# sota-zk-labs/zkp-implementation

Measured on AMD Instinct MI355X. Metric: G1 MSM scalar-muls/sec, higher is better.
Workload: dtype u32 (unsaturated 28-bit-limb Montgomery, 381-bit Fq; 64-bit accumulate)

## Files before the change

zkp-implementation_amd/csrc/api.hip:

```cpp
#include <hip/hip_runtime.h>

#include <algorithm>
#include <array>
#include <atomic>
#include <chrono>
#include <cstdio>
#include <cstdlib>
#include <cstring>
#include <condition_variable>
#include <functional>
#include <map>
#include <memory>
#include <mutex>
#include <new>
#include <string>
#include <thread>
#include <tuple>
#include <vector>

#include "../../include/zkp_hip.h"
#include "host_ff.hpp"
#include "kzg_host.hpp"
#include "msm.hpp"
#include "ntt.hpp"
// ... 225 lines not shown
    Stream stream;
    Stream copy_stream;
    Stream sort_stream;
    Stream xstream;
    Event ws_event;
    hipStream_t ws_stream = nullptr;
    bool ws_pending = false;
    std::vector<ProfRec> prof;
    hipStream_t prof_last = nullptr;
    std::map<std::pair<int, int>, DevBuf> radix_tw[2];
    std::map<std::pair<unsigned, int>, NttPlan<Fr>> plans_fr;
    std::map<std::pair<unsigned, int>, NttPlan<Gl>> plans_gl;
    static constexpr int COSET_WAYS = 8;
    CosetCache<Fr> coset_fr[COSET_WAYS];
    CosetCache<Gl> coset_gl[COSET_WAYS];
    unsigned coset_victim[2] = {0, 0};
    DevBuf ntt_scratch;
    std::map<std::pair<unsigned, int>, DevBuf> axis0_tw[2];
    DevBuf scalars, over;
    TypedBuf<uint32_t> digits, sorted, counts, start, perm, result;
    TypedBuf<uint2> entries;
    TypedBuf<uint4> pieces, buckets, parts, pyr1, odd0, odd1;
    PinnedBuf host_result;
    PinnedBuf fri_small;
    DevBuf fb_table;
    bool fb_ready = false;
    DevBuf tmp;
    Event copy_event;
    std::vector<Event> copy_events;
    Event ev_sort[2], ev_acc[2], ev_begin;
    DevBuf fri_arena, fri_meta;
    DevBuf clk;
    uint32_t tail_max_waves = 2048;
    DevBuf xchg_a, xchg_b;
    std::vector<Event> xev;
    bool peers_enabled = false;
    ~Ctx() {
        std::lock_guard<std::mutex> lk(mu);
        (void)hipSetDevice(device);
        (void)hipDeviceSynchronize();
    }
};
enum { CLK_MSM_ACCUMULATE = 0, CLK_MAD_PROBE = 1, CLK_NTT_FR = 2, CLK_NTT_GL = 3, CLK_COUNT = 4 };
static const char* const kClkNames[CLK_COUNT] = {"msm_accumulate", "mad_probe", "ntt_fr_pass", "ntt_gl_pass"};

struct Runtime {
    std::mutex mu;
    std::vector<std::unique_ptr<Ctx>> slots;
    bool multi = false;
};
Runtime& g_rt = *new Runtime;

ClkRec* clk_record(int which) {
    if (!g_prof_on.load(std::memory_order_relaxed)) return nullptr;
    Ctx& c = ctx();
    if (!c.clk.p) {
        if (c.clk.ensure(sizeof(ClkRec) * CLK_COUNT) != ZKP_OK) return nullptr;
        if (hipMemset(c.clk.p, 0, sizeof(ClkRec) * CLK_COUNT) != hipSuccess) return nullptr;
    }
    return reinterpret_cast<ClkRec*>(c.clk.p) + which;
}
thread_local int t_slot = -1;
thread_local Ctx* t_cur = nullptr;
Ctx& ctx() { return *t_cur; }
std::vector<ProfRec>& prof_records() { return ctx().prof; }
hipStream_t& prof_last_stream() { return ctx().prof_last; }
// ... 640 lines not shown
            cnt++;
        }
    }
    *total_ms = tot;
    *count = cnt;
    return ZKP_OK;
} ZKP_CATCH_INT
const char* zkp_last_error(void) { return g_err.c_str(); }

}

namespace {

int create_slot_locked(int device) {
    int count = 0;
    if (hipGetDeviceCount(&count) != hipSuccess || count == 0) return fail(ZKP_E_DEVICE, "no HIP device visible");
    if (device < 0 || device >= count) return fail(ZKP_E_ARG, "device index out of range");
    hipDeviceProp_t prop;
    HIPCHK(hipGetDeviceProperties(&prop, device));
    if (std::strncmp(prop.gcnArchName, "gfx950", 6) != 0)
        return fail(ZKP_E_DEVICE, std::string("device is ") + prop.gcnArchName + ", this library is built for gfx950 only");
    HIPCHK(hipSetDevice(device));
    ZCHK(allow_big_lds((ntt_pass_strided<Fr, NttOps<Fr>::LOG_T>)));
    ZCHK(allow_big_lds((ntt_pass_strided<Fr, NttOps<Fr>::LOG_T - 1>)));
    ZCHK(allow_big_lds((ntt_pass_strided<Fr, NttOps<Fr>::LOG_T - 2>)));
    ZCHK(allow_big_lds((ntt_pass_strided<Gl, NttOps<Gl>::LOG_T>)));
    ZCHK(allow_big_lds(ntt_pass_last<Fr>));
    ZCHK(allow_big_lds(ntt_pass_last<Gl>));
    ZCHK(allow_big_lds(msm_partscatter_kernel<PS_TILE_BIG>));
    ZCHK(allow_big_lds(msm_partscatter_kernel<PS_TILE_MID>));
    ZCHK(allow_big_lds(msm_partscatter_kernel<PS_TILE_SMALL>));
    ZCHK(allow_big_lds(fri_tail_kernel<FriGl>));
    ZCHK(allow_big_lds(fri_tail_kernel<FriFr>));
    auto c = std::make_unique<Ctx>();
    c->device = device;
    c->slot = (int)g_rt.slots.size();
    {
        int per_cu = 0;
        uint32_t cap = (uint32_t)prop.multiProcessorCount * 4 * 2;
        if (hipOccupancyMaxActiveBlocksPerMultiprocessor(&per_cu, msm_pyramid_tail_kernel, (int)PYR_TAIL_THREADS, 0) == hipSuccess && per_cu > 0)
            cap = std::min<uint32_t>(cap, (uint32_t)per_cu * (uint32_t)prop.multiProcessorCount * (PYR_TAIL_THREADS / 64));
        else
            (void)hipGetLastError();
        c->tail_max_waves = std::max<uint32_t>(cap, 4);
    }
    if (c->stream.make(hipStreamNonBlocking) != hipSuccess) return fail(ZKP_E_DEVICE, "hipStreamCreate failed");
    g_rt.slots.push_back(std::move(c));
    return ZKP_OK;
}

}

extern "C" {

int zkp_init(int device) try {
    std::lock_guard<std::mutex> g(g_rt.mu);
    if (!g_rt.slots.empty()) return ZKP_OK;
    if (device < 0 && hipGetDevice(&device) != hipSuccess) device = 0;
    return create_slot_locked(device);
} ZKP_CATCH_INT

int zkp_init_devices(const int* devices, int n_devices) try {
    if (n_devices < 0 || n_devices > 64) return fail(ZKP_E_ARG, "n_devices out of range");
    std::lock_guard<std::mutex> g(g_rt.mu);
    std::vector<int> want;
    if (n_devices == 0 || !devices) {
        int count = 0;
        if (hipGetDeviceCount(&count) != hipSuccess || count == 0) return fail(ZKP_E_DEVICE, "no HIP device visible");
// ... 756 lines not shown
```

zkp-implementation_amd/csrc/g1_28.hpp:

```cpp
#pragma once
#include "fq28.hpp"

namespace zkp {

struct A28 {
    Fq28 x, y;
    static ZKP_DEV A28 load(const uint4* p) {
        A28 a;
        a.x = Fq28::load(p);
        a.y = Fq28::load(p + 4);
        return a;
    }
    ZKP_DEV void store(uint4* p) const {
        x.store(p);
        y.store(p + 4);
    }
};

struct X28 {
    Fq28 x, y, zz, zzz;
    static ZKP_DEV X28 infinity() {
        X28 r;
        r.x = Fq28::zero(); r.y = Fq28::zero(); r.zz = Fq28::zero(); r.zzz = Fq28::zero();
        return r;
// ... 232 lines not shown
}
template <bool CHAIN = false>
ZKP_DEV void g1_28_add_stream(const uint4* __restrict__ pa, const uint4* __restrict__ pb, uint4* __restrict__ dst, uint64_t st) {
    g1_28_add_stream_body<CHAIN>(pa, pb, dst, st);
}
template <bool CHAIN = false>
ZKP_DEV void g1_28_add_stream_inplace(uint4* pa, const uint4* __restrict__ pb, uint64_t st) {
    g1_28_add_stream_body<CHAIN>(pa, pb, pa, st);
}

template <int CTRL>
ZKP_DEV Fq28 quad_perm(const Fq28& v) {
    Fq28 r;
#pragma unroll
    for (int i = 0; i < NL28; i++) r.l[i] = (uint32_t)__builtin_amdgcn_mov_dpp((int)v.l[i], CTRL, 0xf, 0xf, true);
    return r;
}
ZKP_DEV Fq28 quad_bcast(const Fq28& v, int src) {
    switch (src & 3) {
        case 0: return quad_perm<0x00>(v);
        case 1: return quad_perm<0x55>(v);
        case 2: return quad_perm<0xaa>(v);
        default: return quad_perm<0xff>(v);
    }
}
ZKP_DEV Fq28 quad_xor1(const Fq28& v) { return quad_perm<0xb1>(v); }
ZKP_DEV int quad_bcast0(int v) { return __builtin_amdgcn_mov_dpp(v, 0x00, 0xf, 0xf, true); }
ZKP_DEV Fq28 fq28_select(bool c, const Fq28& a, const Fq28& b) {
    Fq28 r;
#pragma unroll
    for (int i = 0; i < NL28; i++) r.l[i] = c ? a.l[i] : b.l[i];
    return r;
}
ZKP_DEV void g1_28_add_quad(const uint4* srcA, const uint4* __restrict__ srcB, uint4* dst, uint64_t stride, int j) {
    const bool odd = (j & 1) != 0, hi = (j & 2) != 0;
    const uint4* mine = odd ? srcB : srcA;
    const uint4* other = odd ? srcA : srcB;
    const int zf = hi ? 12 : 8;
    const Fq28 xy = Fq28::load_s(mine + (hi ? 4 : 0) * stride, stride);
    const Fq28 zo = Fq28::load_s(other + zf * stride, stride);
    const Fq28 zm = Fq28::load_s(mine + zf * stride, stride);
    const int inf_mine = zm.all_zero() ? 1 : 0, inf_other = zo.all_zero() ? 1 : 0;
    const int inf_a = quad_bcast0(inf_mine), inf_b = quad_bcast0(inf_other);
    const Fq28 m1 = xy * zo;
    const Fq28 d = sub4(quad_xor1(m1), m1);
    const Fq28 m2 = fq28_select(odd, zo, d) * fq28_select(odd, zm, d);
    const Fq28 pp = quad_bcast(m2, 0);
    const int p_zero = quad_bcast0(tight_is_zero_mod_p(m2) ? 1 : 0);
    if (inf_a | inf_b | p_zero) {
        if (j == 0) {
            X28 a = X28::load_s(srcA, stride);
            const X28 b = X28::load_s(srcB, stride);
            g1_28_add(a, b);
            a.store_s(dst, stride);
        }
        return;
    }
    const Fq28 u1 = quad_bcast(m1, 0);
    const Fq28 m3 = fq28_select(hi, u1, fq28_select(odd, m2, d)) * pp;
    const Fq28 ppp = quad_bcast(m3, 0);
    const Fq28 s1 = quad_bcast(m1, 2);
    const Fq28 x3 = normalise(sub8w(sub4(m2, ppp), m3 + m3));
    const Fq28 t = sub16(m3, x3);
    const Fq28 lhs4 = fq28_select(hi, fq28_select(odd, m2, d), s1);
    const Fq28 rhs4 = fq28_select(hi && !odd, t, ppp);
    const Fq28 m4 = lhs4 * rhs4;
    const Fq28 v = quad_bcast(m4, 0);
    if (j == 2) {
        x3.store_s(dst, stride);
        normalise(sub4(m4, v)).store_s(dst + 4 * stride, stride);
    } else if (j == 1) {
        m3.store_s(dst + 8 * stride, stride);
    } else if (j == 3) {
        m4.store_s(dst + 12 * stride, stride);
    }
}

}
```

zkp-implementation_amd/csrc/knobs.hpp:

```cpp
#pragma once
#include <climits>
#include <cstdlib>

namespace zkp {

enum Knob {
    KNOB_MSM_C, KNOB_MSM_FEED_RANGES, KNOB_MSM_FEED_FIRST_PCT, KNOB_MSM_FEED_SECOND_PCT, KNOB_MSM_RANGE_LOG, KNOB_MSM_FIRST_PCT,
    KNOB_MSM_NCHUNK, KNOB_SORT_LO_BITS, KNOB_MSM_NO_OVERLAP, KNOB_MSM_SPLIT_LOG,
    KNOB_MSM_PLAN_END,
    KNOB_FOLD_LANE_MIN = KNOB_MSM_PLAN_END, KNOB_PYR_TAIL_THREADS, KNOB_PYR_TAIL_BLOCKS, KNOB_PYR_TAIL_HALF, KNOB_TEST_TAIL_STARVE,
    KNOB_MSM_NO_POLL, KNOB_POOL_NO_WARM, KNOB_MSM_BALANCE_FROM, KNOB_SRS_EXPAND_MAX_BYTES, KNOB_NTT_TW_MATRIX_MAX_LOG,
    KNOB_NTT_NO_WIDE_PASS, KNOB_NTT_SHARD_MIN_LOG, KNOB_PLONK_NO_POLL, KNOB_FRI_ZERO_AS_0, KNOB_FRI_FR_TAIL_LOG,
    KNOB_COUNT
};

enum KnobKind { KNOB_TUNING, KNOB_POLICY, KNOB_TEST_HOOK };
enum KnobForm {
    KNOB_INT,
    KNOB_INT_CLAMP,
    KNOB_INT_REFUSE,
    KNOB_SET,
    KNOB_ONE
};
constexpr long long KNOB_COMPUTED = LLONG_MIN;

struct KnobRow {
    Knob id;
    const char* name;
    KnobKind kind;
    KnobForm form;
    long long lo, hi, dflt;
    const char* doc;
};

constexpr KnobRow kKnobs[KNOB_COUNT] = {
    {KNOB_MSM_C, "ZKP_MSM_C", KNOB_TUNING, KNOB_INT, 8, 16, KNOB_COMPUTED,
     "window bits of an MSM over unexpanded bases (16 from 2048 terms, else 8): profiles/r01_window_sweep.txt"},
    {KNOB_MSM_FEED_RANGES, "ZKP_MSM_FEED_RANGES", KNOB_TUNING, KNOB_INT, 1, 64, 0,
     "host-fed scalars in this many equal ranges (0: the unequal split): profiles/r04_i_host_scalars_unequal_ranges.md"},
    {KNOB_MSM_FEED_FIRST_PCT, "ZKP_MSM_FEED_FIRST_PCT", KNOB_TUNING, KNOB_INT, 0, 90, KNOB_COMPUTED,
     "share of the first host-fed range (25, from 2^21 terms 10; 0: equal ranges): profiles/r04_i_host_scalars_unequal_ranges.md"},
    {KNOB_MSM_FEED_SECOND_PCT, "ZKP_MSM_FEED_SECOND_PCT", KNOB_TUNING, KNOB_INT, 0, 80, KNOB_COMPUTED,
     "share of a second short host-fed range (30 from 2^21 terms, else none): profiles/r05_o_range_handover.md"},
    {KNOB_MSM_RANGE_LOG, "ZKP_MSM_RANGE_LOG", KNOB_TUNING, KNOB_INT, 10, 30, 0,
     "scalar ranges of at most 2^v terms in shared-bucket mode (0: 2^24, or 2^23 above 12 planes): "
     "profiles/r02_a_accumulate_prefetch_and_range_sweep.md"},
    {KNOB_MSM_FIRST_PCT, "ZKP_MSM_FIRST_PCT", KNOB_TUNING, KNOB_INT, 1, 90, 0,
     "resident scalars, single MSM: a short first range of this share (0: none): profiles/r05_o_range_handover.md"},
    {KNOB_MSM_NCHUNK, "ZKP_MSM_NCHUNK", KNOB_TUNING, KNOB_INT, 1, 4096, 0, "chunks per bucket set of the counting sort (0: 512 over the bucket sets)"},
    {KNOB_SORT_LO_BITS, "ZKP_SORT_LO_BITS", KNOB_TUNING, KNOB_INT, 6, 10, 0,
     "bins of the sort's second pass, 2^v (0: 8..10 by window width): profiles/r04_m_sort_tiles.md"},
    {KNOB_MSM_NO_OVERLAP, "ZKP_MSM_NO_OVERLAP", KNOB_TUNING, KNOB_SET, 0, 1, 0,
     "sort of range r+1 after, not under, the accumulate of range r: profiles/r02_j_sort_under_accumulate.md"},
    {KNOB_MSM_SPLIT_LOG, "ZKP_MSM_SPLIT_LOG", KNOB_TUNING, KNOB_INT, 0, 2, KNOB_COMPUTED,
     "2^v lanes (quads) share a bucket's run in a single-range MSM (default: by bucket count): profiles/r02_n_split_runs.md"},
    {KNOB_FOLD_LANE_MIN, "ZKP_FOLD_LANE_MIN", KNOB_TUNING, KNOB_INT, 0, LLONG_MAX, 1ll << 15,
     "adds in one fold launch from which one lane per add is used: profiles/r05_m_fold_lane.md"},
    {KNOB_PYR_TAIL_THREADS, "ZKP_PYR_TAIL_THREADS", KNOB_TUNING, KNOB_INT_REFUSE, 64, 512, 256,
     "workgroup size of the bucket reduction's last-levels launch, a multiple of 64: profiles/r04_e_bucket_reduce_counters.md"},
    {KNOB_PYR_TAIL_BLOCKS, "ZKP_PYR_TAIL_BLOCKS", KNOB_TUNING, KNOB_INT_REFUSE, 1, 256, 16,
     "workgroups per bucket set of that launch: profiles/r04_e_bucket_reduce_counters.md"},
    {KNOB_PYR_TAIL_HALF, "ZKP_PYR_TAIL_HALF", KNOB_TUNING, KNOB_INT_REFUSE, 1, UINT_MAX, 64,
     "pairs per array from which that launch takes over: profiles/r04_e_bucket_reduce_counters.md"},
    {KNOB_TEST_TAIL_STARVE, "ZKP_TEST_TAIL_STARVE", KNOB_TEST_HOOK, KNOB_SET, 0, 1, 0,
     "every MSM FAILS: the last-levels barrier waits for a workgroup that does not exist (tests/test_gpu_parity.py)"},
    {KNOB_MSM_NO_POLL, "ZKP_MSM_NO_POLL", KNOB_TUNING, KNOB_SET, 0, 1, 0,
     "stream wait instead of polling the MSM's result flags: profiles/r05_k_result_flag_polling.md"},
    {KNOB_POOL_NO_WARM, "ZKP_POOL_NO_WARM", KNOB_TUNING, KNOB_SET, 0, 1, 0,
     "do not wake the host pool before a batch's tails: profiles/r05_q_host_pool_warm.md"},
    {KNOB_MSM_BALANCE_FROM, "ZKP_MSM_BALANCE_FROM", KNOB_TUNING, KNOB_INT, 0, INT_MAX, 1,
     "expansion: slices of floor/ceil(256 / planes) bits from this many bits of overshoot: profiles/r03_j_balanced_slices.md"},
    {KNOB_SRS_EXPAND_MAX_BYTES, "ZKP_SRS_EXPAND_MAX_BYTES", KNOB_POLICY, KNOB_INT, 0, LLONG_MAX, LLONG_MAX,
     "an SRS expansion larger than this is refused with ZKP_E_NOMEM; the bases stay unexpanded"},
    {KNOB_NTT_TW_MATRIX_MAX_LOG, "ZKP_NTT_TW_MATRIX_MAX_LOG", KNOB_TUNING, KNOB_INT_CLAMP, 0, 30, 24,
     "largest transform whose pass-0 twiddles are kept as a matrix: profiles/r02_m_ntt_twiddle_matrix.md"},
    {KNOB_NTT_NO_WIDE_PASS, "ZKP_NTT_NO_WIDE_PASS", KNOB_TUNING, KNOB_SET, 0, 1, 0,
     "no radix-2^9 / 2^10 passes in transform plans built from now on (a plan is cached per size): profiles/r02_l_ntt_wide_pass.md"},
    {KNOB_NTT_SHARD_MIN_LOG, "ZKP_NTT_SHARD_MIN_LOG", KNOB_POLICY, KNOB_INT_CLAMP, 4, INT_MAX, 24,
     "host transforms from 2^v elements are spread over the device slots"},
    {KNOB_PLONK_NO_POLL, "ZKP_PLONK_NO_POLL", KNOB_TUNING, KNOB_SET, 0, 1, 0,
     "stream wait instead of the polled sequence number behind a proof's read-backs: profiles/r05_q_host_pool_warm.md"},
    {KNOB_FRI_ZERO_AS_0, "ZKP_FRI_ZERO_AS_0", KNOB_POLICY, KNOB_ONE, 0, 1, 0,
     "1: a zero field element enters hashes and the transcript as \"0\" instead of the empty string"},
    {KNOB_FRI_FR_TAIL_LOG, "ZKP_FRI_FR_TAIL_LOG", KNOB_TUNING, KNOB_INT_CLAMP, 0, 10, 9,
     "FRI over Fr: layers of up to 2^v points run in the tail kernel (0: none)"},
};

constexpr bool knob_rows_in_enum_order() {
    for (int i = 0; i < KNOB_COUNT; i++)
        if (kKnobs[i].id != i) return false;
    return true;
}
static_assert(knob_rows_in_enum_order(), "kKnobs: one row per enumerator, in the enum's order");

inline long long knob_int(Knob k, long long dflt) {
    const KnobRow& r = kKnobs[k];
// ... 15 lines not shown
```

zkp-implementation_amd/csrc/msm.hpp:

```cpp
#pragma once
#include "g1.hpp"
#include "g1_28.hpp"
#include "fq28_inv.hpp"
#include "msm_plan.hpp"

namespace zkp {

constexpr int MSM_THREADS = 256;
constexpr int ACC_THREADS = 256;
#define ZKP_AT(f, o) offsetof(MsmGeom, f) == o
static_assert(sizeof(MsmGeom) == 152 && ZKP_AT(c, 0) && ZKP_AT(nwin, 4) && ZKP_AT(nb, 8) && ZKP_AT(nchunk, 12) && ZKP_AT(n, 16) && ZKP_AT(chunk, 24) &&
              ZKP_AT(ns, 32) && ZKP_AT(plane_stride, 40) && ZKP_AT(nslice, 48) && ZKP_AT(shared, 52) && ZKP_AT(run_limit, 56) && ZKP_AT(piece, 60) &&
              ZKP_AT(resume, 64) && ZKP_AT(off, 68) && ZKP_AT(interleave, 140) && ZKP_AT(split_log, 144) && ZKP_AT(more, 148), "MsmGeom layout");
#undef ZKP_AT
static_assert(sizeof(SortGeom) == 8 && offsetof(SortGeom, lo_bits) == 0 && offsetof(SortGeom, nhi) == 4, "SortGeom layout");

ZKP_DEV uint64_t bucket_cap(const MsmGeom& g) { return (uint64_t)g.nwin * g.nb; }

#ifdef ZKP_MSM_CHECK
__device__ uint32_t g_msm_check[32];
ZKP_DEV bool msm_check_fail(int cls, uint32_t v0, uint32_t v1) {
    if (atomicAdd(&g_msm_check[cls * 4], 1u) == 0) { g_msm_check[cls * 4 + 1] = v0; g_msm_check[cls * 4 + 2] = v1; }
    return true;
}
// ... 424 lines not shown
        raw.store(planes + (s * plane_stride + i) * 8);
        run.store(slot(s, 2));
        x.zz.store(slot(s, 0));
        x.zzz.store(slot(s, 1));
        run = run * x.zzz;
    }
    Fq28 inv = fq28_inverse_gcd(run);
#pragma unroll 1
    for (uint32_t s = nplanes - 1; s >= 1; s--) {
        const Fq28 zi3 = inv * Fq28::load(slot(s, 2));
        inv = inv * Fq28::load(slot(s, 1));
        const Fq28 zi = zi3 * Fq28::load(slot(s, 0));
        const Fq28 zi2 = zi * zi;
        uint4* dst = planes + (s * plane_stride + i) * 8;
        const A28 raw = A28::load(dst);
        A28 q;
        q.x = raw.x * zi2;
        q.y = raw.y * zi3;
        q.store(dst);
    }
}

ZKP_DEV uint4* split_dst(const MsmGeom& g, uint4* buckets, uint4* parts, uint32_t part) {
    return part ? parts + (uint64_t)(part - 1) * 16 * bucket_cap(g) : buckets;
}
ZKP_DEV void split_run(const MsmGeom& g, uint32_t part, uint32_t& lo, uint32_t& hi) {
    if (!g.split_log) return;
    const uint32_t len = hi - lo;
    hi = lo + (uint32_t)(((uint64_t)len * (part + 1)) >> g.split_log);
    lo = lo + (uint32_t)(((uint64_t)len * part) >> g.split_log);
}


ZKP_DEV uint64_t pyr_pos(uint32_t i, uint32_t n) { return (uint64_t)(i >> 1) + (uint64_t)(i & 1u) * (n >> 1); }

#ifdef ZKP_ACC_PLAIN_PRODUCTS
constexpr bool ACC_CHAIN = false;
#else
constexpr bool ACC_CHAIN = true;
#endif
ZKP_DEV void msm_accumulate_run(const uint4* __restrict__ bases28, const uint32_t* __restrict__ idx, uint32_t lo,
                                uint32_t hi, const MsmGeom& g, uint4* dst, uint64_t dst_stride, bool resume,
                                const uint4* src = nullptr, uint64_t src_stride = 1) {
#ifdef ZKP_MSM_CHECK
    if ((lo > hi || hi > g.n) && msm_check_fail(3, lo, hi)) return;
#endif
    if (resume && lo == hi) {
        if (src != dst) X28::load_s(src, src_stride).store_s(dst, dst_stride);
        return;
    }
    X28 acc = resume ? X28::load_s(src, src_stride) : X28::infinity();
    auto locate = [&](uint32_t e) {
        uint64_t pt = e & 0x7fffffffu;
#ifdef ZKP_MSM_CHECK
        if (pt >= g.n && msm_check_fail(2, e, (uint32_t)g.n)) pt = 0;
#endif
        if (g.shared) {
            const uint32_t ns32 = (uint32_t)g.ns, s = (uint32_t)pt / ns32;
            pt = (uint64_t)s * g.plane_stride + ((uint32_t)pt - s * ns32);
        }
        return bases28 + pt * 8;
    };
    uint32_t k = lo;
    if (!resume && hi - lo >= 2) {
        const uint32_t e0 = idx[k], e1 = idx[k + 1];
        {
            A28 p0 = A28::load(locate(e0));
// ... 249 lines not shown
    const uint4* pw = pieces + (uint64_t)w * desc_cap * 16;
    X28 acc = X28::infinity();
    for (uint32_t p = p0 + lane; p < p1; p += 64) {
        X28 x = X28::load(pw + (uint64_t)p * 16);
        g1_28_add(acc, x);
    }
    for (uint32_t off = 32; off > 0; off >>= 1) {
        acc.store(sh + lane * 16);
        __syncthreads();
        if (lane < off) {
            X28 x = X28::load(sh + (lane + off) * 16);
            g1_28_add(acc, x);
        }
        __syncthreads();
    }
    if (lane == 0) {
        const uint64_t e = (uint64_t)w * g.nb + pyr_pos(b - 1, g.nb);
        if (g.resume) {
            X28 x = X28::load_s(carry + e * 16, 1);
            g1_28_add(acc, x);
        }
        if (g.more) acc.store_s(carry + e * 16, 1);
        else acc.store_s(buckets + e, bucket_cap(g));
    }
    __syncthreads();
    }
}

struct PyrLevel {
    uint32_t level;
    uint32_t half;
    uint32_t nb;
    uint32_t nwin;
};
ZKP_DEV uint64_t odd_off(uint32_t nb, uint32_t j) { return (uint64_t)nb - (nb >> j); }
struct PyrItem {
    uint64_t a, b, d;
    bool src_is_pyr_out;
};
ZKP_DEV PyrItem pyr_item(uint32_t nb, uint32_t level, uint32_t half, uint32_t kind, uint32_t s, uint64_t wbase) {
    PyrItem it;
    if (kind == 0) {
        it.a = wbase + s;
        it.b = wbase + half + s;
        it.d = wbase + pyr_pos(s, half);
        it.src_is_pyr_out = false;
    } else {
        const uint64_t o = wbase + odd_off(nb, kind - 1);
        it.src_is_pyr_out = kind == level;
        const uint64_t src = it.src_is_pyr_out ? wbase + 2 * (uint64_t)half : o;
        it.a = src + s;
        it.b = src + half + s;
        it.d = o + s;
    }
    return it;
}

__global__ __launch_bounds__(MSM_THREADS) void msm_pyramid_kernel(const uint4* __restrict__ pyr_in,
                                                                  uint4* pyr_out,
                                                                  const uint4* __restrict__ odd_in,
                                                                  uint4* __restrict__ odd_out, PyrLevel L) {
    const uint32_t s = blockIdx.x * MSM_THREADS + threadIdx.x;
    if (s >= L.half) return;
    const uint32_t kind = blockIdx.y, w = blockIdx.z;
    const uint64_t cap = (uint64_t)L.nwin * L.nb;
    const PyrItem it = pyr_item(L.nb, L.level, L.half, kind, s, (uint64_t)w * L.nb);
    const uint4* src = kind == 0 ? pyr_in : (it.src_is_pyr_out ? pyr_out : odd_in);
    g1_28_add_stream<ACC_CHAIN>(src + it.a, src + it.b, (kind ? odd_out : pyr_out) + it.d, cap);
}

__global__ __launch_bounds__(MSM_THREADS) void msm_pyramid_quad_kernel(const uint4* __restrict__ pyr_in,
                                                                       uint4* pyr_out,
                                                                       const uint4* __restrict__ odd_in,
                                                                       uint4* __restrict__ odd_out, PyrLevel L) {
    const uint32_t s = blockIdx.x * (MSM_THREADS / 4) + (threadIdx.x >> 2);
    const int j = threadIdx.x & 3;
    if (s >= L.half) return;
    const uint32_t kind = blockIdx.y, w = blockIdx.z;
    const uint64_t cap = (uint64_t)L.nwin * L.nb;
    const PyrItem it = pyr_item(L.nb, L.level, L.half, kind, s, (uint64_t)w * L.nb);
    const uint4* src = kind == 0 ? pyr_in : (it.src_is_pyr_out ? pyr_out : odd_in);
    g1_28_add_quad(src + it.a, src + it.b, (kind ? odd_out : pyr_out) + it.d, cap, j);
}

constexpr uint32_t MSM_TAIL_TIMEOUT = 0x80000000u;
constexpr uint32_t MSM_FLAG_PENDING = 0x40000000u;
constexpr uint32_t MSM_FLAG_PENDING_MASK = 0x40000000u;
constexpr uint32_t PYR_TAIL_THREADS = 256;
constexpr uint32_t PYR_TAIL_BLOCKS = 16;
constexpr uint32_t PYR_TAIL_SPIN_LIMIT = 1u << 24;
__global__ __launch_bounds__(512) void msm_pyramid_tail_kernel(uint4* __restrict__ pyr0, uint4* __restrict__ pyr1,
                                                               uint4* __restrict__ odd0, uint4* __restrict__ odd1,
                                                               uint32_t level0, uint32_t c, uint32_t nb,
                                                               uint32_t* __restrict__ barrier ,
                                                               uint4* __restrict__ result ,
                                                               uint32_t* __restrict__ flags ,
                                                               uint32_t expect_blocks ,
                                                               uint32_t spin_limit) {
    const uint32_t w = blockIdx.y;
    const uint64_t wbase = (uint64_t)w * nb;
    const uint64_t cap = (uint64_t)gridDim.y * nb;
    const int j = threadIdx.x & 3;
    const uint32_t quad = blockIdx.x * (blockDim.x >> 2) + (threadIdx.x >> 2), nquad = gridDim.x * (blockDim.x >> 2);
    uint32_t epoch = 0;
    for (uint32_t l = level0; l + 1 < c; l++) {
        const uint32_t half = nb >> (l + 1);
        const uint4* pyr_in = (l & 1) ? pyr1 : pyr0;
        uint4* pyr_out = (l & 1) ? pyr0 : pyr1;
        const uint4* odd_in = (l & 1) ? odd1 : odd0;
        uint4* odd_out = (l & 1) ? odd0 : odd1;
        for (uint32_t item = quad; item < (l + 1) * half; item += nquad) {
            const uint32_t kind = item / half, s = item % half;
            const PyrItem it = pyr_item(nb, l, half, kind, s, wbase);
            const uint4* src = kind == 0 ? pyr_in : (it.src_is_pyr_out ? pyr_out : odd_in);
            g1_28_add_quad(src + it.a, src + it.b, (kind ? odd_out : pyr_out) + it.d, cap, j);
        }
        epoch++;
        __syncthreads();
        if (threadIdx.x == 0) {
            uint32_t* bar = barrier + (uint64_t)w * PYR_BAR_STRIDE;
            __builtin_amdgcn_fence(__ATOMIC_RELEASE, "agent");
            __hip_atomic_fetch_add(bar, 1u, __ATOMIC_RELAXED, __HIP_MEMORY_SCOPE_AGENT);
            bool arrived = false;
            for (uint32_t spin = 0; spin < spin_limit; spin++) {
                if (__hip_atomic_load(bar, __ATOMIC_RELAXED, __HIP_MEMORY_SCOPE_AGENT) >= epoch * expect_blocks) {
                    arrived = true;
                    break;
                }
                __builtin_amdgcn_s_sleep(1);
            }
            if (!arrived) __hip_atomic_fetch_or(bar, MSM_TAIL_TIMEOUT, __ATOMIC_RELAXED, __HIP_MEMORY_SCOPE_AGENT);
            __builtin_amdgcn_fence(__ATOMIC_ACQUIRE, "agent");
        }
        __syncthreads();
    }
    if (blockIdx.x == 0) {
        const uint4* pyr_final = ((c - 1) & 1) ? pyr1 : pyr0;
        const uint4* pyr_prev = ((c - 1) & 1) ? pyr0 : pyr1;
        const uint4* odd_final = ((c - 1) & 1) ? odd1 : odd0;
        for (uint32_t t = threadIdx.x; t < c * 16; t += blockDim.x) {
            const uint32_t e = t >> 4, q = t & 15;
            const uint4* src = e == 0 ? pyr_final + wbase : e == c - 1 ? pyr_prev + (wbase + 1) : odd_final + (wbase + odd_off(nb, e - 1));
            result[((uint64_t)w * c + e) * 16 + q] = src[q * cap];
        }
        __threadfence_system();
        __syncthreads();
// ... 77 lines not shown
```

zkp-implementation_amd/csrc/msm_host.inc:

```

#ifdef ZKP_MSM_CHECK
#define MSM_TRACE(stream, ridx, what) do { hipError_t e_ = hipStreamSynchronize(stream); fprintf(stderr, "ZKP_MSM_CHECK range %llu: %s done (%d)\n", (unsigned long long)(ridx), what, (int)e_); } while (0)
#else
#define MSM_TRACE(stream, ridx, what) do { } while (0)
#endif

struct MsmFeed {
    const uint64_t* h_scalars;
    hipStream_t copy_stream;
    hipEvent_t ev;
    MsmFeedRanges ranges;
};

struct RangeBuffers {
    uint32_t *sorted, *start, *perm;
    uint4* desc;
    uint32_t *over, *over_b, *over_off;
};

struct MsmPass {
    const MsmPlan& p;
    MsmGeom g;
    const zkp_bases* bases;
    const Fr* const* scalars;
// ... 155 lines not shown
        const uint4* xy = static_cast<const uint4*>(bases->d_xy.p) + off * 8;
        uint4 *buckets = cx.buckets.get(), *pieces = cx.pieces.get(), *parts = cx.parts.get(), *carry = cx.pyr1.get();
        if (quad)
            hipLaunchKernelGGL(msm_accumulate_quad_kernel, grid, dim3(ACC_THREADS), 0, st, xy, rb.sorted, rb.start, rb.perm, rb.over, rb.desc,
                               p.desc_cap, bucket_blocks, extra_blocks, g, buckets, pieces, parts, clk_record(CLK_MSM_ACCUMULATE));
        else
            hipLaunchKernelGGL(msm_accumulate_kernel, grid, dim3(ACC_THREADS), 0, st, xy, rb.sorted, rb.start, rb.perm, rb.over, rb.desc,
                               p.desc_cap, bucket_blocks, extra_blocks, g, buckets, pieces, parts, carry, clk_record(CLK_MSM_ACCUMULATE));
        MSM_TRACE(st, ridx, "accumulate");
        hipLaunchKernelGGL(msm_combine_kernel, dim3(std::min<uint32_t>(p.over_cap, 64), g.nwin), dim3(64), 0, st, rb.over, rb.over_b,
                           rb.over_off, p.over_cap, p.desc_cap, g, pieces, buckets, carry);
        MSM_TRACE(st, ridx, "combine");
        const uint64_t cap = (uint64_t)g.nwin * g.nb;
        const uint64_t lane_from = (uint64_t)knob_int(KNOB_FOLD_LANE_MIN);
        for (uint32_t t = 0; t < g.split_log; t++) {
            const unsigned pairs = 1u << (g.split_log - 1 - t), per = cap * pairs >= lane_from ? MSM_THREADS : MSM_THREADS / 4;
            hipLaunchKernelGGL(per == MSM_THREADS ? msm_fold_parts_lane_kernel : msm_fold_parts_kernel, dim3((unsigned)((cap + per - 1) / per), pairs),
                               dim3(MSM_THREADS), 0, st, buckets, parts, cap, t);
        }
    }

    int reduce() {
        static_assert(kKnobs[KNOB_PYR_TAIL_THREADS].dflt == PYR_TAIL_THREADS && kKnobs[KNOB_PYR_TAIL_BLOCKS].dflt == PYR_TAIL_BLOCKS, "knobs.hpp");
        const uint32_t tail_threads = (uint32_t)knob_int(KNOB_PYR_TAIL_THREADS), tail_blocks = (uint32_t)knob_int(KNOB_PYR_TAIL_BLOCKS);
        const uint32_t tail_half = (uint32_t)knob_int(KNOB_PYR_TAIL_HALF);
        if (tail_threads < 64 || tail_threads > 512 || (tail_threads & 63) || !tail_blocks || tail_blocks > 256 || !tail_half)
            return fail(ZKP_E_ARG, "ZKP_PYR_TAIL_THREADS must be a multiple of 64 up to 512, ZKP_PYR_TAIL_BLOCKS 1..256, ZKP_PYR_TAIL_HALF >= 1");
        for (size_t w = 0; w < W; w++) __atomic_store_n(result_flags + w, MSM_FLAG_PENDING, __ATOMIC_RELEASE);
        uint4* pyr[2] = {cx.buckets.get(), cx.pyr1.get()};
        uint4* odd[2] = {cx.odd0.get(), cx.odd1.get()};
        ProfScope ps("msm_bucket_reduce", st, true);
        uint32_t level_tail = 0;
        while (level_tail + 1 < g.c && (g.nb >> (level_tail + 1)) > tail_half) level_tail++;
        const uint32_t max_waves = cx.tail_max_waves;
        if ((uint64_t)g.nwin * (tail_threads / 64) > max_waves) level_tail = g.c - 1;
        for (uint32_t l = 0; l < level_tail; l++) {
            const PyrLevel L{l, g.nb >> (l + 1), g.nb, g.nwin};
            const bool quad = (uint64_t)L.half * (l + 1) * g.nwin <= (1u << 16);
            const uint32_t per = quad ? MSM_THREADS / 4 : MSM_THREADS;
            hipLaunchKernelGGL(quad ? msm_pyramid_quad_kernel : msm_pyramid_kernel, dim3((L.half + per - 1) / per, l + 1, g.nwin),
                               dim3(MSM_THREADS), 0, st, pyr[l & 1], pyr[(l + 1) & 1], odd[l & 1], odd[(l + 1) & 1], L);
        }
        if (level_tail + 1 < g.c) {
            uint32_t tb = tail_blocks;
            while (tb > 1 && (uint64_t)tb * g.nwin * (tail_threads / 64) > max_waves) tb >>= 1;
            const bool starve = knob_flag(KNOB_TEST_TAIL_STARVE);
            hipLaunchKernelGGL(msm_pyramid_tail_kernel, dim3(tb, g.nwin), dim3(tail_threads), 0, st, pyr[0], pyr[1], odd[0], odd[1], level_tail,
                               g.c, g.nb, cx.result.get(), result_out, result_flags, starve ? tb + 1 : tb, starve ? (1u << 12) : PYR_TAIL_SPIN_LIMIT);
        } else {
            const uint32_t fin = (g.c - 1) & 1;
            hipLaunchKernelGGL(msm_collect_kernel, dim3(g.nwin), dim3(64), 0, st, pyr[fin], pyr[fin ^ 1], odd[fin], g.nb, g.c, result_out,
                               result_flags);
        }
        return ZKP_OK;
    }
};

int wait_msm_result(const MsmGeom& g, const uint32_t* flags, hipStream_t st) {
    ZCHK(poll_or_sync(g.n <= (1ull << 24) && !knob_flag(KNOB_MSM_NO_POLL), st, [&] {
        for (size_t w = 0; w < g.nwin; w++)
            if (__atomic_load_n(flags + w, __ATOMIC_ACQUIRE) & MSM_FLAG_PENDING) return false;
        return true;
    }));
    for (size_t w = 0; w < g.nwin; w++)
        if (flags[w] & MSM_TAIL_TIMEOUT)
            return fail(ZKP_E_DEVICE, "bucket reduction: the workgroups of the last levels did not all become resident (device shared "
                                      "with another job?); no result was produced");
    return ZKP_OK;
}

void msm_host_tail(const uint32_t* host_res, size_t count, uint32_t wins_per_msm, uint32_t c, HXyzz* out) {
    const auto t_tail0 = std::chrono::steady_clock::now();
    auto tail = [&](size_t m) {
        const uint32_t* res = host_res + m * wins_per_msm * c * 64;
        HXyzz total = HXyzz::infinity();
        for (int pos = (int)(wins_per_msm * c) - 1; pos >= 0; pos--) {
            total = total.dbl();
            const int w = pos / (int)c, l = pos % (int)c;
            const uint32_t* rw = res + (size_t)w * c * 64;
            if (l <= (int)c - 2) total = total.add(xyzz_from_internal(rw + (size_t)(1 + l) * 64));
            if (l == 0) total = total.add(xyzz_from_internal(rw));
// ... 52 lines not shown
```

zkp-implementation_amd/csrc/msm_plan.hpp:

```cpp
#pragma once
#include <algorithm>
#include <cstddef>
#include <cstdint>
#include <cstdlib>
#include <vector>

#include "../../include/zkp_hip.h"
#include "knobs.hpp"

namespace zkp {

struct MsmGeom {
    uint32_t c;
    uint32_t nwin;
    uint32_t nb;
    uint32_t nchunk;
    uint64_t n;
    uint64_t chunk;
    uint64_t ns;
    uint64_t plane_stride;
    uint32_t nslice;
    uint32_t shared;
    uint32_t run_limit;
    uint32_t piece;
    uint32_t resume;
    uint16_t off[36];
    uint32_t interleave;
    uint32_t split_log;
    uint32_t more;
};

struct SortGeom {
    uint32_t lo_bits;
    uint32_t nhi;
};

constexpr int MSM_MAX_BATCH = 64;
constexpr uint32_t SORT_MAX_PART = 8192;
constexpr uint32_t MSM_MAX_WINDOW_BITS = 24;
constexpr uint32_t PYR_BAR_STRIDE = 32;
constexpr uint64_t SPLIT_FILL_LANES = 6 * 1024 * 64, SPLIT_FILL_QUADS = 2 * 1024 * 64 / 4 * 2;
// ... 84 lines not shown
    if (g.n >= (1ull << 31)) return refuse(ZKP_E_ARG, "windows x scalars >= 2^31 with expanded bases");
    g.nb = 1u << (g.c - 1);
    g.interleave = (g.nwin > 1 && g.n <= (1ull << 22)) ? 1u : 0u;
    const uint64_t entries = g.n;
    g.nchunk = (uint32_t)std::min<uint64_t>(std::max<uint32_t>(1, (512 + g.nwin - 1) / g.nwin), (entries + 4095) / 4096);
    if (const long long v = knob_int(KNOB_MSM_NCHUNK)) g.nchunk = (uint32_t)std::min<uint64_t>((uint64_t)v, entries);
    g.chunk = (entries + g.nchunk - 1) / g.nchunk;
    g.run_limit = (uint32_t)std::max<uint64_t>(128, 4 * (entries / g.nb));
    g.piece = (uint32_t)std::max<uint64_t>(32, entries / g.nb);
    SortGeom& sg = p->sg;
    sg.lo_bits = std::min<uint32_t>(g.c >= 21 ? 10 : g.c >= 20 ? 9 : 8, g.c - 1);
    if (const long long lo = knob_int(KNOB_SORT_LO_BITS); lo && (uint32_t)lo < g.c) sg.lo_bits = (uint32_t)lo;
    sg.nhi = g.nb >> sg.lo_bits;
    if (sg.nhi > SORT_MAX_PART) return refuse(ZKP_E_ARG, "window width above 24 bits is not supported by the sort");
    const size_t W = g.nwin, nb = g.nb, c = g.c;
    p->overlap = shared && range < n && !knob_flag(KNOB_MSM_NO_OVERLAP);
    const size_t nbuf = p->nbuf = p->overlap ? 2 : 1;
    p->over_cap = (uint32_t)std::min<uint64_t>(entries / 128 + 1, (uint64_t)nb);
    p->desc_cap = (uint32_t)(entries / g.piece + entries / g.run_limit + 2);
    p->over_bytes = ((4 * W * (2 + (size_t)p->over_cap + p->over_cap + 1) + 16 * W * (size_t)p->desc_cap) + 255) & ~(size_t)255;
    const uint64_t units = (uint64_t)nb * W;
    const uint64_t want_units = (uint64_t)g.n * g.nwin <= (1ull << 20) ? SPLIT_FILL_QUADS : SPLIT_FILL_LANES;
    if (range >= n) {
        while (g.split_log < MSM_MAX_SPLIT_LOG && (units << g.split_log) < want_units) g.split_log++;
        g.split_log = (uint32_t)knob_int(KNOB_MSM_SPLIT_LOG, g.split_log);
    }
    p->bytes = MsmSizes{4 * W * entries, nbuf * 4 * W * entries, 4 * W * ((size_t)g.nchunk * sg.nhi + 2 * sg.nhi + 1 + 512),
                        8 * W * entries, nbuf * 4 * W * (nb + 2), nbuf * 4 * W * nb, nbuf * p->over_bytes,
                        256 * W * (size_t)p->desc_cap, 256 * W * nb, 256 * W * nb * ((1u << g.split_log) - 1),
                        256 * W * nb, 256 * W * nb, 256 * W * nb, 4 * PYR_BAR_STRIDE * W, 256 * W * c + 4 * W};
    return ZKP_OK;
}

}
```

Baseline: 440.9 million.

## Fuse narrow bucket-reduction pyramid levels into workgroup-local LDS subtrees

Adds a workgroup-local pyramid kernel that runs several consecutive narrow levels of the bucket reduction in LDS (up to 160 KiB per group), writing only the final level back to global memory. A host-side schedule picks a level span when a cost model predicts fewer rounds than launching each level on its own. The aim is to cut per-level launch overhead and global round-trips during the narrow levels that underfill the GPU. The cost is extra index bookkeeping ('born_in_odd' layout), big LDS allocations that limit occupancy, and a knob to turn the feature off.

```diff
diff --git a/zkp-implementation_amd/csrc/api.hip b/zkp-implementation_amd/csrc/api.hip
--- a/zkp-implementation_amd/csrc/api.hip
+++ b/zkp-implementation_amd/csrc/api.hip
@@ -281,6 +281,7 @@
     DevBuf fri_arena, fri_meta;
     DevBuf clk;
     uint32_t tail_max_waves = 2048;
+    uint32_t cus = 256;
     DevBuf xchg_a, xchg_b;
     std::vector<Event> xev;
     bool peers_enabled = false;
@@ -987,8 +988,10 @@
     ZCHK(allow_big_lds(msm_partscatter_kernel<PS_TILE_SMALL>));
     ZCHK(allow_big_lds(fri_tail_kernel<FriGl>));
     ZCHK(allow_big_lds(fri_tail_kernel<FriFr>));
+    ZCHK(allow_big_lds(msm_pyramid_local_kernel));
     auto c = std::make_unique<Ctx>();
     c->device = device;
+    c->cus = (uint32_t)std::max(prop.multiProcessorCount, 1);
     c->slot = (int)g_rt.slots.size();
     {
         int per_cu = 0;
diff --git a/zkp-implementation_amd/csrc/g1_28.hpp b/zkp-implementation_amd/csrc/g1_28.hpp
--- a/zkp-implementation_amd/csrc/g1_28.hpp
+++ b/zkp-implementation_amd/csrc/g1_28.hpp
@@ -288,7 +288,7 @@
     for (int i = 0; i < NL28; i++) r.l[i] = c ? a.l[i] : b.l[i];
     return r;
 }
-ZKP_DEV void g1_28_add_quad(const uint4* srcA, const uint4* __restrict__ srcB, uint4* dst, uint64_t stride, int j) {
+ZKP_DEV void g1_28_add_quad_body(const uint4* srcA, const uint4* srcB, uint64_t stride, uint4* dst, uint64_t dstride, int j) {
     const bool odd = (j & 1) != 0, hi = (j & 2) != 0;
     const uint4* mine = odd ? srcB : srcA;
     const uint4* other = odd ? srcA : srcB;
@@ -308,7 +308,7 @@
             X28 a = X28::load_s(srcA, stride);
             const X28 b = X28::load_s(srcB, stride);
             g1_28_add(a, b);
-            a.store_s(dst, stride);
+            a.store_s(dst, dstride);
         }
         return;
     }
@@ -323,13 +323,16 @@
     const Fq28 m4 = lhs4 * rhs4;
     const Fq28 v = quad_bcast(m4, 0);
     if (j == 2) {
-        x3.store_s(dst, stride);
-        normalise(sub4(m4, v)).store_s(dst + 4 * stride, stride);
+        x3.store_s(dst, dstride);
+        normalise(sub4(m4, v)).store_s(dst + 4 * dstride, dstride);
     } else if (j == 1) {
-        m3.store_s(dst + 8 * stride, stride);
+        m3.store_s(dst + 8 * dstride, dstride);
     } else if (j == 3) {
-        m4.store_s(dst + 12 * stride, stride);
-    }
-}
-
-}
+        m4.store_s(dst + 12 * dstride, dstride);
+    }
+}
+ZKP_DEV void g1_28_add_quad(const uint4* srcA, const uint4* __restrict__ srcB, uint4* dst, uint64_t stride, int j) {
+    g1_28_add_quad_body(srcA, srcB, stride, dst, stride, j);
+}
+
+}
diff --git a/zkp-implementation_amd/csrc/knobs.hpp b/zkp-implementation_amd/csrc/knobs.hpp
--- a/zkp-implementation_amd/csrc/knobs.hpp
+++ b/zkp-implementation_amd/csrc/knobs.hpp
@@ -8,7 +8,7 @@
     KNOB_MSM_C, KNOB_MSM_FEED_RANGES, KNOB_MSM_FEED_FIRST_PCT, KNOB_MSM_FEED_SECOND_PCT, KNOB_MSM_RANGE_LOG, KNOB_MSM_FIRST_PCT,
     KNOB_MSM_NCHUNK, KNOB_SORT_LO_BITS, KNOB_MSM_NO_OVERLAP, KNOB_MSM_SPLIT_LOG,
     KNOB_MSM_PLAN_END,
-    KNOB_FOLD_LANE_MIN = KNOB_MSM_PLAN_END, KNOB_PYR_TAIL_THREADS, KNOB_PYR_TAIL_BLOCKS, KNOB_PYR_TAIL_HALF, KNOB_TEST_TAIL_STARVE,
+    KNOB_FOLD_LANE_MIN = KNOB_MSM_PLAN_END, KNOB_PYR_TAIL_THREADS, KNOB_PYR_TAIL_BLOCKS, KNOB_PYR_TAIL_HALF, KNOB_PYR_NO_LOCAL, KNOB_TEST_TAIL_STARVE,
     KNOB_MSM_NO_POLL, KNOB_POOL_NO_WARM, KNOB_MSM_BALANCE_FROM, KNOB_SRS_EXPAND_MAX_BYTES, KNOB_NTT_TW_MATRIX_MAX_LOG,
     KNOB_NTT_NO_WIDE_PASS, KNOB_NTT_SHARD_MIN_LOG, KNOB_PLONK_NO_POLL, KNOB_FRI_ZERO_AS_0, KNOB_FRI_FR_TAIL_LOG,
     KNOB_COUNT
@@ -62,6 +62,8 @@
      "workgroups per bucket set of that launch: profiles/r04_e_bucket_reduce_counters.md"},
     {KNOB_PYR_TAIL_HALF, "ZKP_PYR_TAIL_HALF", KNOB_TUNING, KNOB_INT_REFUSE, 1, UINT_MAX, 64,
      "pairs per array from which that launch takes over: profiles/r04_e_bucket_reduce_counters.md"},
+    {KNOB_PYR_NO_LOCAL, "ZKP_PYR_NO_LOCAL", KNOB_TUNING, KNOB_SET, 0, 1, 0,
+     "every narrow level of the bucket reduction as its own launch, none as workgroup-local subtrees: profiles/r06_a_pyramid_local.md"},
     {KNOB_TEST_TAIL_STARVE, "ZKP_TEST_TAIL_STARVE", KNOB_TEST_HOOK, KNOB_SET, 0, 1, 0,
      "every MSM FAILS: the last-levels barrier waits for a workgroup that does not exist (tests/test_gpu_parity.py)"},
     {KNOB_MSM_NO_POLL, "ZKP_MSM_NO_POLL", KNOB_TUNING, KNOB_SET, 0, 1, 0,
diff --git a/zkp-implementation_amd/csrc/msm.hpp b/zkp-implementation_amd/csrc/msm.hpp
--- a/zkp-implementation_amd/csrc/msm.hpp
+++ b/zkp-implementation_amd/csrc/msm.hpp
@@ -480,7 +480,6 @@
 }
 
 
-ZKP_DEV uint64_t pyr_pos(uint32_t i, uint32_t n) { return (uint64_t)(i >> 1) + (uint64_t)(i & 1u) * (n >> 1); }
 
 #ifdef ZKP_ACC_PLAIN_PRODUCTS
 constexpr bool ACC_CHAIN = false;
@@ -796,29 +795,8 @@
     uint32_t half;
     uint32_t nb;
     uint32_t nwin;
+    uint32_t born_in_odd;
 };
-ZKP_DEV uint64_t odd_off(uint32_t nb, uint32_t j) { return (uint64_t)nb - (nb >> j); }
-struct PyrItem {
-    uint64_t a, b, d;
-    bool src_is_pyr_out;
-};
-ZKP_DEV PyrItem pyr_item(uint32_t nb, uint32_t level, uint32_t half, uint32_t kind, uint32_t s, uint64_t wbase) {
-    PyrItem it;
-    if (kind == 0) {
-        it.a = wbase + s;
-        it.b = wbase + half + s;
-        it.d = wbase + pyr_pos(s, half);
-        it.src_is_pyr_out = false;
-    } else {
-        const uint64_t o = wbase + odd_off(nb, kind - 1);
-        it.src_is_pyr_out = kind == level;
-        const uint64_t src = it.src_is_pyr_out ? wbase + 2 * (uint64_t)half : o;
-        it.a = src + s;
-        it.b = src + half + s;
-        it.d = o + s;
-    }
-    return it;
-}
 
 __global__ __launch_bounds__(MSM_THREADS) void msm_pyramid_kernel(const uint4* __restrict__ pyr_in,
                                                                   uint4* pyr_out,
@@ -828,7 +806,7 @@
     if (s >= L.half) return;
     const uint32_t kind = blockIdx.y, w = blockIdx.z;
     const uint64_t cap = (uint64_t)L.nwin * L.nb;
-    const PyrItem it = pyr_item(L.nb, L.level, L.half, kind, s, (uint64_t)w * L.nb);
+    const PyrItem it = pyr_item(L.nb, L.level, L.half, kind, s, (uint64_t)w * L.nb, L.born_in_odd != 0);
     const uint4* src = kind == 0 ? pyr_in : (it.src_is_pyr_out ? pyr_out : odd_in);
     g1_28_add_stream<ACC_CHAIN>(src + it.a, src + it.b, (kind ? odd_out : pyr_out) + it.d, cap);
 }
@@ -842,9 +820,46 @@
     if (s >= L.half) return;
     const uint32_t kind = blockIdx.y, w = blockIdx.z;
     const uint64_t cap = (uint64_t)L.nwin * L.nb;
-    const PyrItem it = pyr_item(L.nb, L.level, L.half, kind, s, (uint64_t)w * L.nb);
+    const PyrItem it = pyr_item(L.nb, L.level, L.half, kind, s, (uint64_t)w * L.nb, L.born_in_odd != 0);
     const uint4* src = kind == 0 ? pyr_in : (it.src_is_pyr_out ? pyr_out : odd_in);
     g1_28_add_quad(src + it.a, src + it.b, (kind ? odd_out : pyr_out) + it.d, cap, j);
+}
+
+__global__ __launch_bounds__(PYR_LOCAL_THREADS) void msm_pyramid_local_kernel(uint4* pyr0, uint4* pyr1, uint4* odd0, uint4* odd1,
+                                                                             PyrLocal P) {
+    extern __shared__ uint4 pyr_lds[];
+    const uint32_t k = blockIdx.x, w = blockIdx.y;
+    const uint32_t nb = P.nb, l0 = P.l0, m = P.m;
+    const uint64_t wbase = (uint64_t)w * nb, cap = (uint64_t)gridDim.y * nb, S = P.lds_stride;
+    uint4* const pyr_in = (l0 & 1) ? pyr1 : pyr0;
+    uint4* const pyr_other = (l0 & 1) ? pyr0 : pyr1;
+    uint4* const odd_in = (l0 & 1) ? odd1 : odd0;
+    uint4* const odd_out = (l0 & 1) ? odd0 : odd1;
+    auto at = [&](uint32_t space, uint64_t e) -> uint4* {
+        switch (space) {
+            case PYR_SP_LDS: return pyr_lds + e;
+            case PYR_SP_PYR_IN: return pyr_in + (wbase + e);
+            case PYR_SP_PYR_OTHER: return pyr_other + (wbase + e);
+            case PYR_SP_ODD_IN: return odd_in + (wbase + e);
+            default: return odd_out + (wbase + e);
+        }
+    };
+    const int j = threadIdx.x & 3;
+    const uint32_t quad = threadIdx.x >> 2, nquad = PYR_LOCAL_THREADS / 4;
+    for (uint32_t t = 0; t < m; t++) {
+        const uint32_t hh = P.block >> (t + 1);
+        for (uint32_t item = quad; item < (l0 + t + 1) * hh; item += nquad) {
+            const PyrLocalItem it = pyr_local_item(P, k, t, item / hh, item % hh);
+            g1_28_add_quad_body(at(it.src, it.a), at(it.src, it.b), it.src == PYR_SP_LDS ? S : cap, at(it.dst, it.d),
+                                it.dst == PYR_SP_LDS ? S : cap, j);
+        }
+        __syncthreads();
+    }
+    const PyrLocalItem born = pyr_local_born(P, k);
+    const uint4* src = pyr_lds + born.a;
+    uint4* dst = odd_out + (wbase + born.d);
+    const uint32_t r = (uint32_t)born.b;
+    for (uint32_t x = threadIdx.x; x < r * 16; x += PYR_LOCAL_THREADS) dst[(x / r) * cap + x % r] = src[(x / r) * S + x % r];
 }
 
 constexpr uint32_t MSM_TAIL_TIMEOUT = 0x80000000u;
@@ -860,7 +875,8 @@
                                                                uint4* __restrict__ result ,
                                                                uint32_t* __restrict__ flags ,
                                                                uint32_t expect_blocks ,
-                                                               uint32_t spin_limit) {
+                                                               uint32_t spin_limit,
+                                                               uint32_t born_in_odd ) {
     const uint32_t w = blockIdx.y;
     const uint64_t wbase = (uint64_t)w * nb;
     const uint64_t cap = (uint64_t)gridDim.y * nb;
@@ -875,7 +891,7 @@
         uint4* odd_out = (l & 1) ? odd0 : odd1;
         for (uint32_t item = quad; item < (l + 1) * half; item += nquad) {
             const uint32_t kind = item / half, s = item % half;
-            const PyrItem it = pyr_item(nb, l, half, kind, s, wbase);
+            const PyrItem it = pyr_item(nb, l, half, kind, s, wbase, l == level0 && born_in_odd);
             const uint4* src = kind == 0 ? pyr_in : (it.src_is_pyr_out ? pyr_out : odd_in);
             g1_28_add_quad(src + it.a, src + it.b, (kind ? odd_out : pyr_out) + it.d, cap, j);
         }
diff --git a/zkp-implementation_amd/csrc/msm_host.inc b/zkp-implementation_amd/csrc/msm_host.inc
--- a/zkp-implementation_amd/csrc/msm_host.inc
+++ b/zkp-implementation_amd/csrc/msm_host.inc
@@ -211,21 +211,37 @@
         ProfScope ps("msm_bucket_reduce", st, true);
         uint32_t level_tail = 0;
         while (level_tail + 1 < g.c && (g.nb >> (level_tail + 1)) > tail_half) level_tail++;
-        const uint32_t max_waves = cx.tail_max_waves;
+        uint32_t max_waves = cx.tail_max_waves;
+        if (tail_threads != PYR_TAIL_THREADS) {
+            int per_cu = 0;
+            if (hipOccupancyMaxActiveBlocksPerMultiprocessor(&per_cu, msm_pyramid_tail_kernel, (int)tail_threads, 0) == hipSuccess && per_cu > 0)
+                max_waves = std::min<uint32_t>(max_waves, std::max<uint32_t>((uint32_t)per_cu * cx.cus * (tail_threads / 64), 4));
+            else
+                (void)hipGetLastError();
+        }
         if ((uint64_t)g.nwin * (tail_threads / 64) > max_waves) level_tail = g.c - 1;
-        for (uint32_t l = 0; l < level_tail; l++) {
-            const PyrLevel L{l, g.nb >> (l + 1), g.nb, g.nwin};
-            const bool quad = (uint64_t)L.half * (l + 1) * g.nwin <= (1u << 16);
+        const PyrSchedule sch = pyr_schedule(g.nb, g.c, g.nwin, cx.cus, level_tail, !knob_flag(KNOB_PYR_NO_LOCAL));
+        for (const PyrStep& s : sch.steps) {
+            if (s.local.m) {
+                hipLaunchKernelGGL(msm_pyramid_local_kernel, dim3(s.local.groups, g.nwin), dim3(PYR_LOCAL_THREADS), pyr_local_lds_bytes(s.local),
+                                   st, pyr[0], pyr[1], odd[0], odd[1], s.local);
+                continue;
+            }
+            const uint32_t l = s.level;
+            const PyrLevel L{l, g.nb >> (l + 1), g.nb, g.nwin, s.born_in_odd};
+            const bool quad = (uint64_t)L.half * (l + 1) * g.nwin <= PYR_QUAD_MAX_ITEMS;
             const uint32_t per = quad ? MSM_THREADS / 4 : MSM_THREADS;
             hipLaunchKernelGGL(quad ? msm_pyramid_quad_kernel : msm_pyramid_kernel, dim3((L.half + per - 1) / per, l + 1, g.nwin),
                                dim3(MSM_THREADS), 0, st, pyr[l & 1], pyr[(l + 1) & 1], odd[l & 1], odd[(l + 1) & 1], L);
         }
+        level_tail = sch.level_tail;
         if (level_tail + 1 < g.c) {
             uint32_t tb = tail_blocks;
             while (tb > 1 && (uint64_t)tb * g.nwin * (tail_threads / 64) > max_waves) tb >>= 1;
             const bool starve = knob_flag(KNOB_TEST_TAIL_STARVE);
             hipLaunchKernelGGL(msm_pyramid_tail_kernel, dim3(tb, g.nwin), dim3(tail_threads), 0, st, pyr[0], pyr[1], odd[0], odd[1], level_tail,
-                               g.c, g.nb, cx.result.get(), result_out, result_flags, starve ? tb + 1 : tb, starve ? (1u << 12) : PYR_TAIL_SPIN_LIMIT);
+                               g.c, g.nb, cx.result.get(), result_out, result_flags, starve ? tb + 1 : tb, starve ? (1u << 12) : PYR_TAIL_SPIN_LIMIT,
+                               sch.tail_born_in_odd);
         } else {
             const uint32_t fin = (g.c - 1) & 1;
             hipLaunchKernelGGL(msm_collect_kernel, dim3(g.nwin), dim3(64), 0, st, pyr[fin], pyr[fin ^ 1], odd[fin], g.nb, g.c, result_out,
diff --git a/zkp-implementation_amd/csrc/msm_plan.hpp b/zkp-implementation_amd/csrc/msm_plan.hpp
--- a/zkp-implementation_amd/csrc/msm_plan.hpp
+++ b/zkp-implementation_amd/csrc/msm_plan.hpp
@@ -7,6 +7,12 @@
 
 #include "../../include/zkp_hip.h"
 #include "knobs.hpp"
+
+#if defined(__HIPCC__)
+#define ZKP_PLAN_HD __host__ __device__ inline
+#else
+#define ZKP_PLAN_HD inline
+#endif
 
 namespace zkp {
 
@@ -157,4 +163,129 @@
     return ZKP_OK;
 }
 
-}
+constexpr uint32_t PYR_LOCAL_THREADS = 256;
+constexpr uint32_t PYR_LOCAL_LDS_BYTES = 160 * 1024;
+constexpr uint32_t PYR_QUAD_MAX_ITEMS = 1u << 16;
+struct PyrLocal {
+    uint32_t l0, m;
+    uint32_t nb;
+    uint32_t groups;
+    uint32_t block;
+    uint32_t lds_stride;
+    uint32_t born_in_odd;
+};
+ZKP_PLAN_HD uint64_t pyr_pos(uint32_t i, uint32_t n) { return (uint64_t)(i >> 1) + (uint64_t)(i & 1u) * (n >> 1); }
+ZKP_PLAN_HD uint64_t odd_off(uint32_t nb, uint32_t j) { return (uint64_t)nb - (nb >> j); }
+struct PyrItem {
+    uint64_t a, b, d;
+    bool src_is_pyr_out;
+};
+ZKP_PLAN_HD PyrItem pyr_item(uint32_t nb, uint32_t level, uint32_t half, uint32_t kind, uint32_t s, uint64_t wbase, bool born_in_odd = false) {
+    PyrItem it;
+    if (kind == 0) {
+        it.a = wbase + s;
+        it.b = wbase + half + s;
+        it.d = wbase + pyr_pos(s, half);
+        it.src_is_pyr_out = false;
+    } else {
+        const uint64_t o = wbase + odd_off(nb, kind - 1);
+        it.src_is_pyr_out = kind == level && !born_in_odd;
+        const uint64_t src = it.src_is_pyr_out ? wbase + 2 * (uint64_t)half : o;
+        it.a = src + s;
+        it.b = src + half + s;
+        it.d = o + s;
+    }
+    return it;
+}
+
+enum PyrSpace : uint32_t { PYR_SP_LDS, PYR_SP_PYR_IN, PYR_SP_PYR_OTHER, PYR_SP_ODD_IN, PYR_SP_ODD_OUT };
+struct PyrLocalItem { uint32_t src, dst; uint64_t a, b, d; };
+ZKP_PLAN_HD uint32_t pyr_local_level(const PyrLocal& P, uint32_t t) {
+    const uint32_t h = P.block >> 1;
+    return P.l0 * h + (h >> 1) + ((t & 1) ? 0u : h);
+}
+ZKP_PLAN_HD uint32_t pyr_local_home(const PyrLocal& P, uint32_t j) {
+    const uint32_t h = P.block >> 1;
+    return j <= P.l0 ? j * h : pyr_local_level(P, j - P.l0) + (h >> (j - P.l0));
+}
+ZKP_PLAN_HD PyrLocalItem pyr_local_item(const PyrLocal& P, uint32_t k, uint32_t t, uint32_t kind, uint32_t i) {
+    const uint32_t l0 = P.l0, B = P.block, h = B >> 1, n0 = P.nb >> l0, half0 = n0 >> 1, hh = B >> (t + 1), j = kind - 1;
+    PyrLocalItem it;
+    it.src = PYR_SP_LDS;
+    if (kind == 0) {
+        if (t == 0) it.src = PYR_SP_PYR_IN, it.a = (uint64_t)k * h + i, it.b = it.a + half0;
+        else it.a = pyr_local_level(P, t) + i, it.b = it.a + hh;
+    } else {
+        if (t == 0 && kind == l0 && !P.born_in_odd) it.src = PYR_SP_PYR_OTHER, it.a = (uint64_t)n0 + (uint64_t)k * B + i;
+        else if (t == 0) it.src = PYR_SP_ODD_IN, it.a = odd_off(P.nb, j) + (uint64_t)k * B + i;
+        else if (t == 1 && j == l0) it.src = PYR_SP_PYR_IN, it.a = (uint64_t)half0 + (uint64_t)k * h + i;
+        else it.a = pyr_local_home(P, j) + i;
+        it.b = it.a + hh;
+    }
+    if (t + 1 == P.m) {
+        it.dst = kind == 0 ? PYR_SP_PYR_OTHER : PYR_SP_ODD_OUT;
+        it.d = kind == 0 ? pyr_pos(k * hh + i, n0 >> P.m) : odd_off(P.nb, j) + (uint64_t)k * hh + i;
+    } else {
+        it.dst = PYR_SP_LDS;
+        it.d = kind == 0 ? pyr_local_level(P, t + 1) + pyr_pos(i, hh) : pyr_local_home(P, j) + i;
+    }
+    return it;
+}
+ZKP_PLAN_HD PyrLocalItem pyr_local_born(const PyrLocal& P, uint32_t k) {
+    const uint32_t r = P.block >> P.m;
+    return {PYR_SP_LDS, PYR_SP_ODD_OUT, (uint64_t)pyr_local_level(P, P.m - 1) + r, r, odd_off(P.nb, P.l0 + P.m - 1) + (uint64_t)k * r};
+}
+
+inline uint32_t pyr_local_lds_bytes(const PyrLocal& L) { return 256 * L.lds_stride; }
+inline uint32_t pyr_local_rounds(uint32_t l0, uint32_t m, uint32_t block) {
+    uint32_t r = 0;
+    for (uint32_t t = 0; t < m; t++) r += ((l0 + t + 1) * (block >> (t + 1)) + PYR_LOCAL_THREADS / 4 - 1) / (PYR_LOCAL_THREADS / 4);
+    return r;
+}
+inline PyrLocal pyr_local_plan(uint32_t nb, uint32_t c, uint32_t nwin, uint32_t l0, uint32_t cus) {
+    PyrLocal best{l0, 0, nb, 0, 0, 0, 0};
+    const uint32_t n0 = nb >> l0, per_round = PYR_LOCAL_THREADS / 4;
+    if (!cus || !nwin || (uint64_t)(n0 >> 1) * (l0 + 1) * nwin > PYR_QUAD_MAX_ITEMS) return best;
+    uint32_t gmax = 1;
+    while ((uint64_t)gmax * 2 * nwin <= cus) gmax *= 2;
+    long best_gain = 1;
+    for (uint32_t m = 3; m <= 7 && l0 + m + 2 <= c; m += 2) {
+        if ((n0 >> m) == 0) break;
+        uint32_t groups = std::min(gmax, n0 >> m);
+        auto stride = [&](uint32_t gr) { return (n0 / gr / 2) * (l0 + 2) + 1; };
+        while (256 * (uint64_t)stride(groups) > PYR_LOCAL_LDS_BYTES && groups < (n0 >> m)) groups *= 2;
+        if (256 * (uint64_t)stride(groups) > PYR_LOCAL_LDS_BYTES) continue;
+        const uint32_t block = n0 / groups;
+        const uint64_t turns = ((uint64_t)groups * nwin + cus - 1) / cus;
+        const long local = 1 + (long)(turns * pyr_local_rounds(l0, m, block));
+        long levels = 0;
+        for (uint32_t t = 0; t < m; t++)
+            levels += 1 + (long)(((uint64_t)(n0 >> (t + 1)) * (l0 + t + 1) * nwin + (uint64_t)cus * per_round - 1) / ((uint64_t)cus * per_round));
+        if (levels - local > best_gain) {
+            best_gain = levels - local;
+            best = PyrLocal{l0, m, nb, groups, block, stride(groups), 0};
+        }
+    }
+    return best;
+}
+
+
+struct PyrStep { PyrLocal local; uint32_t level, born_in_odd; };
+struct PyrSchedule { std::vector<PyrStep> steps; uint32_t level_tail, tail_born_in_odd; };
+inline PyrSchedule pyr_schedule(uint32_t nb, uint32_t c, uint32_t nwin, uint32_t cus, uint32_t level_tail, bool local) {
+    PyrSchedule s{{}, 0, 0};
+    uint32_t l = 0, born = 0;
+    while (l + 1 < c) {
+        PyrLocal pl = local ? pyr_local_plan(nb, c, nwin, l, cus) : PyrLocal{};
+        if (!pl.m && l >= level_tail) break;
+        pl.born_in_odd = pl.m ? born : 0;
+        s.steps.push_back({pl, l, born});
+        l += pl.m ? pl.m : 1;
+        born = pl.m ? 1 : 0;
+    }
+    s.level_tail = l;
+    s.tail_born_in_odd = born;
+    return s;
+}
+
+}
```

New measurement: 435.0 million. 1.3% lower.
